# robo-alex/gs-dynamics

Hardware: AMD Instinct MI355X
Metric: fwd+bwd Mpix/s at 100k Gaussians, 4x800^2 views (higher is better)
Workload: dtype f32

## Files before the change

gs-dynamics_amd/csrc/gsr_binning.hip:

```cpp
#include "gsr_common.h"

namespace gsr_binning {

#define SCAN_THREADS 1024
#define SCAN_ITEMS 8
__global__ __launch_bounds__(SCAN_THREADS) void scan_exclusive_kernel(const uint32_t* __restrict__ in,
                                                                      uint32_t* __restrict__ out, uint32_t n,
                                                                      uint32_t* __restrict__ total_out) {
  __shared__ uint32_t wave_tot[SCAN_THREADS / GSR_WAVE];
  __shared__ uint32_t carry_s;
  const int tid = threadIdx.x, lane = tid & 63, wv = tid >> 6;
  if (tid == 0) carry_s = 0;
  __syncthreads();
  const uint32_t per_round = SCAN_THREADS * SCAN_ITEMS;
  for (uint32_t base = 0; base < n; base += per_round) {
    uint32_t v[SCAN_ITEMS];
    uint32_t first = base + (uint32_t)tid * SCAN_ITEMS;
    uint32_t sum = 0;
#pragma unroll
    for (int k = 0; k < SCAN_ITEMS; ++k) {
      uint32_t idx = first + k;
      v[k] = idx < n ? in[idx] : 0u;
      sum += v[k];
    }
// ... 660 lines not shown
  __syncthreads();
  uint32_t before = 0, total = 0;
#pragma unroll
  for (int w = 0; w < GSR_BLOCK / 64; ++w) { if (w < wv) before += s_w[w]; total += s_w[w]; }
  uint32_t* __restrict__ words = vw.block_hist;
  if (tid == 0) __hip_atomic_store(&words[blockIdx.x], 0x80000000u | total, __ATOMIC_RELAXED, __HIP_MEMORY_SCOPE_AGENT);
  if (wv == 0) {
    uint32_t mine = 0;
    if (lane < (int)blockIdx.x) {
      uint32_t w;
      do { w = __hip_atomic_load(&words[lane], __ATOMIC_RELAXED, __HIP_MEMORY_SCOPE_AGENT); } while (!(w & 0x80000000u));
      mine = w & 0x7fffffffu;
    }
#pragma unroll
    for (int k = 32; k >= 1; k >>= 1) mine += __shfl_xor(mine, k, 64);
    if (lane == 0) s_base = mine;
  }
  __syncthreads();
  const uint32_t start = s_base + before + inc - run, cap = vw.D;
  if (t < T) vw.ranges[t] = make_uint2(min(start, cap), min(start + run, cap));
}

__device__ __forceinline__ void bin_scan_view(const GsrBinViews& tab, const GsrBinView& vw, int prefixed, uint32_t* s_wave, uint32_t* s_carry) {
  const int T = tab.T, Ts = gsr_bin_stride(T), rows = tab.rows, tid = threadIdx.x, lane = tid & 63, wv = tid >> 6;
  uint32_t* __restrict__ m = vw.tile_rows;
  const uint32_t cap = vw.D;
  if (tid == 0) *s_carry = 0;
  __syncthreads();
  for (int q0 = 0; q0 < Ts / 4; q0 += BIN_THREADS) {
    const int q = q0 + tid;
    const bool live = q < Ts / 4;
    uint4 tot = make_uint4(0u, 0u, 0u, 0u);
    if (live) {
      if (prefixed) tot = *reinterpret_cast<const uint4*>(m + (size_t)rows * Ts + 4 * q);
      else {
        for (int r0 = 0; r0 < rows; r0 += BIN_ROW_CHUNK) {
          uint4 v[BIN_ROW_CHUNK];
#pragma unroll
          for (int r = 0; r < BIN_ROW_CHUNK; ++r)
            v[r] = r0 + r < rows ? *reinterpret_cast<const uint4*>(m + (size_t)(r0 + r) * Ts + 4 * q) : make_uint4(0u, 0u, 0u, 0u);
#pragma unroll
          for (int r = 0; r < BIN_ROW_CHUNK; ++r)
            if (r0 + r < rows) {
              *reinterpret_cast<uint4*>(m + (size_t)(r0 + r) * Ts + 4 * q) = tot;
              tot.x += v[r].x; tot.y += v[r].y; tot.z += v[r].z; tot.w += v[r].w;
            }
        }
      }
    }
    const uint32_t mine = tot.x + tot.y + tot.z + tot.w;
    uint32_t inc = mine;
#pragma unroll
    for (int d = 1; d < 64; d <<= 1) {
      const uint32_t o = __shfl_up(inc, d, 64);
      if (lane >= d) inc += o;
    }
    if (lane == 63) s_wave[wv] = inc;
    __syncthreads();
    uint32_t start = *s_carry + inc - mine;
    for (int w = 0; w < wv; ++w) start += s_wave[w];
    if (live) {
      const uint32_t c[4] = {tot.x, tot.y, tot.z, tot.w};
      uint32_t st_ = start;
#pragma unroll
      for (int k = 0; k < 4; ++k) {
        if (4 * q + k < T) vw.ranges[4 * q + k] = make_uint2(min(st_, cap), min(st_ + c[k], cap));
        st_ += c[k];
      }
    }
    __syncthreads();
    if (tid == BIN_THREADS - 1) *s_carry = start + mine;
    __syncthreads();
  }
}

__global__ __launch_bounds__(BIN_THREADS) void bin_scan_kernel(GsrBinViews tab, int prefixed) {
  __shared__ uint32_t s_wave[BIN_THREADS / 64];
  __shared__ uint32_t s_carry;
  const GsrBinView& vw = tab.v[blockIdx.x];
  if (vw.shares_lists) return;
  bin_scan_view(tab, vw, prefixed, s_wave, &s_carry);
}

__global__ __launch_bounds__(BIN_THREADS) void bin_emit_kernel(int P, GsrBinViews tab, int order_wgs, int items_per_wg) {
  extern __shared__ uint32_t s_cur[];
  if ((int)blockIdx.x >= tab.rows) {
    __shared__ TileOrderLds L;
    if (blockIdx.y == 0) tile_order_body(tab, items_per_wg, (int)blockIdx.x - tab.rows, L);
    return;
  }
  (void)order_wgs;
  __shared__ uint2 s_big[BIN_BIG_MAX];
  __shared__ uint64_t s_bigkey[BIN_BIG_MAX];
  __shared__ uint32_t s_nbig;
  const GsrBinView& vw = tab.v[blockIdx.y];
  const int T = tab.T, Ts = gsr_bin_stride(T), gx = tab.gx, tid = threadIdx.x, lane = tid & 63, wv = tid >> 6;
  const int g0 = (int)blockIdx.x * GSR_BIN_G;
  if (vw.shares_lists) return;
  const uint32_t cap = vw.D;
  const uint32_t* __restrict__ row = vw.tile_rows + (size_t)blockIdx.x * Ts;
  const uint32_t* __restrict__ cut = vw.depth_cut;
  const bool cut_l = cut && tab.cut_lds;
  const uint32_t* s_cut = s_cur + T;
  const uint32_t* s_cc = s_cur + 2 * T;
  const int gxc = (gx + 3) >> 2;
  if (cut_l)
    for (int t = tid; t < T; t += BIN_THREADS) s_cur[T + t] = cut[t];
  auto cut_at = [&](uint32_t t) { return cut_l ? s_cut[t] : cut[t]; };
  auto behind_all = [&](uint2 r, uint32_t dbits) {
    const uint32_t x0 = (r.x & 0xffffu) >> 2, y0 = (r.x >> 16) >> 2, x1 = ((r.y & 0xffffu) - 1u) >> 2, y1 = ((r.y >> 16) - 1u) >> 2;
    uint32_t m = 0u;
    for (uint32_t y = y0; y <= y1; ++y)
      for (uint32_t x = x0; x <= x1; ++x) m = max(m, s_cc[y * gxc + x]);
    return dbits > m;
  };
  uint64_t* __restrict__ dg = vw.dg[0];
  uint2 rc[BIN_PER_THREAD], ek[BIN_PER_THREAD];
#pragma unroll
  for (int q = 0; q < BIN_PER_THREAD; ++q) {
    const int g = g0 + tid * BIN_PER_THREAD + q;
    rc[q] = make_uint2(0u, 0u); ek[q] = rc[q];
    if (g < P) { rc[q] = vw.rect[g]; ek[q] = vw.ekey[g]; }
  }
  if (tid == 0) s_nbig = 0;
  for (int t = tid; t < T; t += BIN_THREADS) s_cur[t] = vw.ranges[t].x + row[t];
  __syncthreads();
  if (cut_l) {
    const int gyc = (T / gx + 3) >> 2;
    for (int c = tid; c < gxc * gyc; c += BIN_THREADS) {
      const int cx = c % gxc, cy = c / gxc;
      uint32_t m = 0u;
      for (int y = 4 * cy; y < min(4 * cy + 4, T / gx); ++y)
        for (int x = 4 * cx; x < min(4 * cx + 4, gx); ++x) m = max(m, s_cut[y * gx + x]);
      s_cur[2 * T + c] = m;
    }
    __syncthreads();
  }
#pragma unroll
  for (int q = 0; q < BIN_PER_THREAD; ++q) {
    const BinGauss b = bin_gauss(rc[q], ek[q].y);
    if (b.area == 0u) continue;
    if (cut_l && behind_all(rc[q], ek[q].x)) continue;
    const uint64_t key = ((uint64_t)ek[q].x << 32) | (uint32_t)(g0 + tid * BIN_PER_THREAD + q);
    if (b.area > BIN_BIG_AREA) {
      const uint32_t slot = atomicAdd(&s_nbig, 1u);
      if (slot < BIN_BIG_MAX) { s_big[slot] = rc[q]; s_bigkey[slot] = key; continue; }
    }
    const uint32_t dbits = ek[q].x;
    bin_for_tiles(b, gx, [&](uint32_t t) {
      if (cut && dbits > cut_at(t)) return;
      const uint32_t slot = atomicAdd(&s_cur[t], 1u);
      if (slot < cap) dg[slot] = key;
    });
  }
  __syncthreads();
  const uint32_t nbig = min(s_nbig, (uint32_t)BIN_BIG_MAX);
  for (uint32_t i = wv; i < nbig; i += BIN_THREADS / 64) {
    const BinGauss b = bin_gauss(s_big[i], 0u);
    const uint64_t key = s_bigkey[i];
    for (uint32_t k = lane; k < b.area; k += 64) {
      const uint32_t t = bin_tile_of(b, k, gx);
      if (cut && (uint32_t)(key >> 32) > cut_at(t)) continue;
      const uint32_t slot = atomicAdd(&s_cur[t], 1u);
      if (slot < cap) dg[slot] = key;
    }
  }
}

__global__ __launch_bounds__(GSR_BLOCK) void tile_ranges_kernel(GsrBinViews tab, int cur) {
  const GsrBinView& vw = tab.v[blockIdx.y];
  const uint32_t* __restrict__ tkey = vw.tkey[cur];
  uint2* __restrict__ ranges = vw.ranges;
  const uint32_t D = bin_entries(vw);
  uint32_t i = blockIdx.x * GSR_BLOCK + threadIdx.x;
  if (i >= D) return;
  uint32_t t = tkey[i];
  if (i == 0) ranges[t].x = 0;
  else {
    uint32_t pt = tkey[i - 1];
    if (pt != t) { ranges[pt].y = i; ranges[t].x = i; }
  }
  if (i == D - 1) ranges[t].y = D;
}


template <typename PTR>
__device__ __forceinline__ void tile_sort_network(PTR a, uint32_t n, int tid, const uint32_t NT = GSR_BLOCK) {
  uint32_t lg = 1;
  while ((1u << lg) < n) ++lg;
  const uint32_t npairs = (1u << lg) >> 1;
  for (uint32_t lk = 1; lk <= lg; ++lk) {
    const uint32_t k = 1u << lk, hk = k >> 1;
    for (uint32_t p = tid; p < npairs; p += NT) {
      const uint32_t base = (p >> (lk - 1)) << lk, off = p & (hk - 1);
      const uint32_t l = base + off, r = base + (k - 1 - off);
      if (r < n) {
        uint64_t x = a[l], y = a[r];
        if (y < x) { a[l] = y; a[r] = x; }
      }
    }
    __syncthreads();
    for (int lj = (int)lk - 2; lj >= 0; --lj) {
      const uint32_t j = 1u << lj;
      for (uint32_t p = tid; p < npairs; p += NT) {
        const uint32_t l = ((p >> lj) << (lj + 1)) + (p & (j - 1)), r = l + j;
        if (r < n) {
          uint64_t x = a[l], y = a[r];
          if (y < x) { a[l] = y; a[r] = x; }
        }
      }
      __syncthreads();
    }
  }
}

template <int M>
__device__ __forceinline__ uint32_t gsr_lane_xor(uint32_t v) {
  if constexpr (M == 1) return (uint32_t)__builtin_amdgcn_update_dpp(0, (int)v, 0xB1, 0xf, 0xf, true);
  else if constexpr (M == 2) return (uint32_t)__builtin_amdgcn_update_dpp(0, (int)v, 0x4E, 0xf, 0xf, true);
  else if constexpr (M == 3) return (uint32_t)__builtin_amdgcn_update_dpp(0, (int)v, 0x1B, 0xf, 0xf, true);
  else if constexpr (M == 7) return (uint32_t)__builtin_amdgcn_update_dpp(0, (int)v, 0x141, 0xf, 0xf, true);
  else if constexpr (M == 15) return (uint32_t)__builtin_amdgcn_update_dpp(0, (int)v, 0x140, 0xf, 0xf, true);
  else if constexpr (M == 8) return (uint32_t)__builtin_amdgcn_update_dpp(0, (int)v, 0x128, 0xf, 0xf, true);
  else if constexpr (M < 32) return (uint32_t)__builtin_amdgcn_ds_swizzle((int)v, (M << 10) | 0x1F);
  else return (uint32_t)__shfl_xor((int)v, M, 64);
}
template <int V> struct gsr_log2 { static constexpr int value = 1 + gsr_log2<(V >> 1)>::value; };
template <> struct gsr_log2<1> { static constexpr int value = 0; };
template <int MASK, int NR>
__device__ __forceinline__ void wave_sort_step(uint64_t (&x)[NR], int lane) {
  constexpr int LR = gsr_log2<NR>::value;
  constexpr int R = MASK & (NR - 1), L = MASK >> LR;
  constexpr int HB = MASK >= 1024 ? 1024 : MASK >= 512 ? 512 : MASK >= 256 ? 256 : MASK >= 128 ? 128 : MASK >= 64 ? 64 : MASK >= 32 ? 32 : MASK >= 16 ? 16 : MASK >= 8 ? 8 : MASK >= 4 ? 4 : MASK >= 2 ? 2 : 1;
  if constexpr (L == 0) {
#pragma unroll
    for (int r = 0; r < NR; ++r) {
      if ((r & HB) == 0) {
        const uint64_t a = x[r], b = x[r ^ R];
        const bool sw = b < a;
        x[r] = sw ? b : a;
        x[r ^ R] = sw ? a : b;
      }
    }
  } else {
    uint64_t y[NR];
#pragma unroll
    for (int r = 0; r < NR; ++r) {
      const uint64_t src = x[r ^ R];
      y[r] = ((uint64_t)gsr_lane_xor<L>((uint32_t)(src >> 32)) << 32) | gsr_lane_xor<L>((uint32_t)src);
    }
    const bool upper = (lane & (HB >> LR)) != 0;
#pragma unroll
    for (int r = 0; r < NR; ++r) {
      const bool take = (y[r] < x[r]) != upper;
      x[r] = take ? y[r] : x[r];
    }
  }
}
template <int LK, int NR>
__device__ __forceinline__ void wave_sort_stage(uint64_t (&x)[NR], int lane) {
  static_assert(LK <= 11, "the half-cleaner steps below stop at stride 512");
  wave_sort_step<(1 << LK) - 1, NR>(x, lane);
  if constexpr (LK >= 11) wave_sort_step<512, NR>(x, lane);
  if constexpr (LK >= 10) wave_sort_step<256, NR>(x, lane);
  if constexpr (LK >= 9) wave_sort_step<128, NR>(x, lane);
  if constexpr (LK >= 8) wave_sort_step<64, NR>(x, lane);
  if constexpr (LK >= 7) wave_sort_step<32, NR>(x, lane);
  if constexpr (LK >= 6) wave_sort_step<16, NR>(x, lane);
  if constexpr (LK >= 5) wave_sort_step<8, NR>(x, lane);
  if constexpr (LK >= 4) wave_sort_step<4, NR>(x, lane);
  if constexpr (LK >= 3) wave_sort_step<2, NR>(x, lane);
  if constexpr (LK >= 2) wave_sort_step<1, NR>(x, lane);
}
template <int NR>
__device__ __forceinline__ void wave_sort_tile(const uint64_t* __restrict__ seg, uint32_t* __restrict__ out, uint32_t n, int lane) {
  uint64_t x[NR];
#pragma unroll
  for (int r = 0; r < NR; ++r) { const uint32_t e = (uint32_t)(r * 64 + lane); x[r] = e < n ? seg[e] : ~0ull; }
  wave_sort_stage<1, NR>(x, lane); wave_sort_stage<2, NR>(x, lane); wave_sort_stage<3, NR>(x, lane);
  wave_sort_stage<4, NR>(x, lane); wave_sort_stage<5, NR>(x, lane); wave_sort_stage<6, NR>(x, lane);
  if constexpr (NR >= 2) wave_sort_stage<7, NR>(x, lane);
  if constexpr (NR >= 4) wave_sort_stage<8, NR>(x, lane);
  if constexpr (NR >= 8) wave_sort_stage<9, NR>(x, lane);
  if constexpr (NR >= 16) wave_sort_stage<10, NR>(x, lane);
  if constexpr (NR >= 32) wave_sort_stage<11, NR>(x, lane);
  const uint32_t e0 = (uint32_t)lane * NR;
  if constexpr (NR >= 4) {
    if ((((uintptr_t)out) & 15u) == 0 && e0 + NR <= n) {
#pragma unroll
      for (int r = 0; r < NR; r += 4)
        *reinterpret_cast<uint4*>(out + e0 + r) = make_uint4((uint32_t)x[r], (uint32_t)x[r + 1], (uint32_t)x[r + 2], (uint32_t)x[r + 3]);
      return;
    }
  }
#pragma unroll
  for (int r = 0; r < NR; ++r) if (e0 + r < n) out[e0 + r] = (uint32_t)x[r];
}

template <int RCAP, int NW = 4>
struct TileSortLds {
  union {
    struct { uint32_t key[2][RCAP]; uint32_t val[2][RCAP]; } r;
    uint64_t net[2 * RCAP];
  };
  uint32_t whist[NW][256];
  uint32_t wtot[4];
  uint32_t diff;
};

template <int RCAP, int NW>
__device__ __forceinline__ int tile_radix_sort(TileSortLds<RCAP, NW>& L, uint32_t n, int tid) {
  constexpr int NT = 64 * NW;
  const int lane = tid & 63, wv = tid >> 6;
  const uint32_t q = ((n + (uint32_t)NT - 1u) / (uint32_t)NT) << 6;
  const uint32_t wstart = min(n, (uint32_t)wv * q), wstop = min(n, wstart + q);
  const uint32_t diff = L.diff;
  int cur = 0;
  for (int shift = 0; shift < 32; shift += 8) {
    if (((diff >> shift) & 0xffu) == 0u) continue;
    const uint32_t* __restrict__ kin = L.r.key[cur];
    const uint32_t* __restrict__ vin = L.r.val[cur];
    uint32_t* __restrict__ kout = L.r.key[cur ^ 1];
    uint32_t* __restrict__ vout = L.r.val[cur ^ 1];
    for (int i = tid; i < NW * 256; i += NT) (&L.whist[0][0])[i] = 0;
    __syncthreads();
    for (uint32_t i = wstart + lane; i < wstop; i += 64) atomicAdd(&L.whist[wv][(kin[i] >> shift) & 0xffu], 1u);
    __syncthreads();
    {
      uint32_t c[NW], tot = 0;
      if (tid < 256) {
#pragma unroll
        for (int w = 0; w < NW; ++w) { c[w] = L.whist[w][tid]; tot += c[w]; }
      }
      uint32_t inc = tot;
#pragma unroll
      for (int d = 1; d < 64; d <<= 1) {
        const uint32_t o = __shfl_up(inc, d, 64);
        if (lane >= d) inc += o;
      }
      if (tid < 256 && lane == 63) L.wtot[wv] = inc;
      __syncthreads();
      if (tid < 256) {
        uint32_t base = inc - tot;
        for (int w = 0; w < wv; ++w) base += L.wtot[w];
#pragma unroll
        for (int w = 0; w < NW; ++w) { L.whist[w][tid] = base; base += c[w]; }
      }
    }
    __syncthreads();
    volatile uint32_t* wbase = L.whist[wv];
    for (uint32_t i0 = wstart; i0 < wstop; i0 += 64) {
      const uint32_t i = i0 + lane;
      const bool valid = i < wstop;
      uint32_t key = 0, val = 0;
      if (valid) { key = kin[i]; val = vin[i]; }
      const uint32_t digit = (key >> shift) & 0xffu;
      const uint64_t peers = match_peers(digit, valid, 8);
      const uint32_t rank = (uint32_t)__popcll(peers & gsr_lanemask_lt());
      uint32_t pos = 0;
      if (valid) pos = wbase[digit] + rank;
      __builtin_amdgcn_wave_barrier();
      if (valid && rank == 0) wbase[digit] = pos + (uint32_t)__popcll(peers);
      __builtin_amdgcn_wave_barrier();
      if (valid) { kout[pos] = key; vout[pos] = val; }
    }
    __syncthreads();
    cur ^= 1;
  }
  return cur;
}

template <int RCAP, int NW>
__device__ __forceinline__ void tile_sort_long_ticket(const GsrBinViews& tab, int cur, uint32_t ticket);

#ifndef TS_W32_WAVES
#define TS_W32_WAVES 5
#endif
#ifndef TS_MIN_WAVES
#define TS_MIN_WAVES 7
#endif
template <int RCAP, int MODE = 0, int NW = 4>
__global__ __launch_bounds__(64 * NW, (RCAP <= 1024 || MODE == 2) ? TS_MIN_WAVES : (MODE == 3 ? TS_W32_WAVES : 1)) void tile_sort_kernel(GsrBinViews tab, int cur) {
  const int tid = threadIdx.x;
  if constexpr (MODE == 3) {
    const uint32_t n_long3 = tab.queue[6], n_mid = tab.queue[3];
    const uint32_t ticket = n_long3 + blockIdx.x * 4u + (uint32_t)(tid >> 6);
    if (ticket >= n_mid) return;
    const uint4 ord = tab.order[ticket];
    const GsrBinView& vw = tab.v[__builtin_amdgcn_readfirstlane(ord.w)];
    if (vw.shares_lists) return;
    const uint32_t n = __builtin_amdgcn_readfirstlane(ord.z - ord.y);
    wave_sort_tile<32>(vw.dg[cur] + ord.y, vw.point_list + ord.y, n, tid & 63);
    return;
  }
  const uint32_t n_busy = tab.queue[4], n_long = tab.queue[6];
  if (MODE == 2 || (MODE == 0 && blockIdx.x >= n_long)) {
    const uint32_t first = (MODE == 2 && tab.wave_cap == 2048) ? tab.queue[3] : n_long;
    const uint32_t ticket = first + (MODE == 2 ? blockIdx.x : blockIdx.x - n_long) * 4u + (uint32_t)(tid >> 6);
    if (ticket >= n_busy) return;
    const uint4 ord = tab.order[ticket];
    const GsrBinView& vw = tab.v[__builtin_amdgcn_readfirstlane(ord.w)];
    if (vw.shares_lists) return;
    const uint32_t n = __builtin_amdgcn_readfirstlane(ord.z - ord.y);
    const uint64_t* seg = vw.dg[cur] + ord.y;
    uint32_t* out = vw.point_list + ord.y;
    if (n <= 64) wave_sort_tile<1>(seg, out, n, tid & 63);
    else if (n <= 128) wave_sort_tile<2>(seg, out, n, tid & 63);
    else if (n <= 256) wave_sort_tile<4>(seg, out, n, tid & 63);
    else if (n <= 512) wave_sort_tile<8>(seg, out, n, tid & 63);
    else wave_sort_tile<16>(seg, out, n, tid & 63);
    return;
  }
  if constexpr (MODE == 1) {
    const uint32_t n_mine = tab.wave_cap == 512 ? tab.queue[2] : n_long;
    for (uint32_t ticket = blockIdx.x; ticket < n_mine; ticket += gridDim.x) {
      tile_sort_long_ticket<RCAP, NW>(tab, cur, ticket);
      __syncthreads();
    }
  } else if constexpr (MODE != 2) {
    if (blockIdx.x >= n_long) return;
    if (RCAP <= 1024 && tab.vlong_launch && blockIdx.x < tab.queue[2]) return;
    tile_sort_long_ticket<RCAP, NW>(tab, cur, blockIdx.x);
  }
}

template <int RCAP, int NW>
__device__ __forceinline__ void tile_sort_long_ticket(const GsrBinViews& tab, int cur, uint32_t ticket) {
  __shared__ TileSortLds<RCAP, NW> L;
  constexpr uint32_t NT = 64 * NW;
  const int tid = threadIdx.x;
  const uint4 ord = tab.order[ticket];
  const GsrBinView& vw = tab.v[__builtin_amdgcn_readfirstlane(ord.w)];
  if (vw.shares_lists) return;
  uint64_t* __restrict__ dg = vw.dg[cur];
  uint32_t* __restrict__ point_list = vw.point_list;
  const uint2 rg = make_uint2(ord.y, ord.z);
  const uint32_t n = rg.y - rg.x;
  if (n == 0) return;
  uint64_t* seg = dg + rg.x;
  if (n == 1) {
    if (tid == 0) point_list[rg.x] = (uint32_t)seg[0];
  } else if (n <= (uint32_t)RCAP) {
    if (tid == 0) L.diff = 0;
    __syncthreads();
    const uint32_t k0 = (uint32_t)(seg[0] >> 32);
    uint32_t d = 0;
    for (uint32_t i = tid; i < n; i += NT) {
      const uint64_t e = seg[i];
      const uint32_t k = (uint32_t)(e >> 32);
      L.r.key[0][i] = k; L.r.val[0][i] = (uint32_t)e;
      d |= k ^ k0;
    }
    if (d) atomicOr(&L.diff, d);
    __syncthreads();
    const int cur = tile_radix_sort(L, n, tid);
    {
      uint32_t* __restrict__ kk = L.r.key[cur];
      uint32_t* __restrict__ vv = L.r.val[cur];
      bool long_run = false;
      for (uint32_t i = tid; i + 1 < n; i += NT) {
        if (kk[i] == kk[i + 1] && (i == 0 || kk[i - 1] != kk[i])) {
          uint32_t j = i + 1;
          while (j + 1 < n && kk[j + 1] == kk[i] && j - i < 32u) ++j;
          if (j + 1 < n && kk[j + 1] == kk[i]) { long_run = true; continue; }
          for (uint32_t a = i + 1; a <= j; ++a) {
            const uint32_t x = vv[a];
            uint32_t b = a;
            while (b > i && vv[b - 1] > x) { vv[b] = vv[b - 1]; --b; }
            vv[b] = x;
          }
        }
      }
      if (__syncthreads_or(long_run ? 1 : 0)) {
        uint64_t e[(RCAP + NT - 1) / NT];
#pragma unroll
        for (int u = 0; u < (RCAP + NT - 1) / NT; ++u) {
          const uint32_t i = (uint32_t)u * NT + tid;
          e[u] = i < n ? (((uint64_t)kk[i] << 32) | vv[i]) : 0ull;
        }
        __syncthreads();
#pragma unroll
        for (int u = 0; u < (RCAP + NT - 1) / NT; ++u) {
          const uint32_t i = (uint32_t)u * NT + tid;
          if (i < n) L.net[i] = e[u];
        }
        __syncthreads();
        tile_sort_network(L.net, n, tid, NT);
        for (uint32_t i = tid; i < n; i += NT) point_list[rg.x + i] = (uint32_t)L.net[i];
        return;
      }
    }
    for (uint32_t i = tid; i < n; i += NT) point_list[rg.x + i] = L.r.val[cur][i];
  } else if (n <= 2u * (uint32_t)RCAP) {
    for (uint32_t i = tid; i < n; i += NT) L.net[i] = seg[i];
    __syncthreads();
    tile_sort_network(L.net, n, tid, NT);
    for (uint32_t i = tid; i < n; i += NT) point_list[rg.x + i] = (uint32_t)L.net[i];
  } else {
    __syncthreads();
    tile_sort_network((volatile uint64_t*)seg, n, tid, NT);
    for (uint32_t i = tid; i < n; i += NT) point_list[rg.x + i] = (uint32_t)seg[i];
  }
}

__global__ __launch_bounds__(GSR_BLOCK) void copy_tile_state_kernel(int T, int n_order, const uint2* __restrict__ src_ranges,
                                                                    const uint4* __restrict__ src_order, const uint32_t* __restrict__ src_queue,
                                                                    uint2* __restrict__ ranges, uint4* __restrict__ order, uint32_t* __restrict__ queue) {
  const int i = blockIdx.x * GSR_BLOCK + threadIdx.x;
  if (i < T) ranges[i] = src_ranges[i];
  if (i < n_order) order[i] = src_order[i];
  if (i < 9) queue[i] = (i == 4 || i == 6 || i == 7) ? src_queue[i] : 0u;
}

}
using namespace gsr_binning;

int gsr_launch_shared_lists(const GsrBinViews& tab_in, int P, uint32_t D, const uint2* owner_ranges, const uint4* owner_order,
                            const uint32_t* owner_queue, uint2* ranges, uint4* order, uint32_t* queue, hipStream_t st) {
  GsrBinViews tab = tab_in;
  tab.v[0].shares_lists = 1;
  { GSR_PROF("emit_entries", st);
    hipLaunchKernelGGL(emit_entries_kernel, dim3(D / GSR_RADIX_EPB + 1u, 1), dim3(GSR_BLOCK), 0, st, P, tab, 0, 1); }
  GSR_HIP_CHECK(hipGetLastError());
  { GSR_PROF("copy_tile_state", st);
    hipLaunchKernelGGL(copy_tile_state_kernel, dim3((tab.T + GSR_BLOCK - 1) / GSR_BLOCK), dim3(GSR_BLOCK), 0, st, tab.T, tab.T, owner_ranges,
                       owner_order, owner_queue, ranges, order, queue); }
  GSR_HIP_CHECK(hipGetLastError());
  return 0;
}

int gsr_launch_scan_exclusive(const uint32_t* in, uint32_t* out, uint32_t n, uint32_t* total_out, hipStream_t st) {
  { GSR_PROF("scan", st);
  hipLaunchKernelGGL(scan_exclusive_kernel, dim3(1), dim3(SCAN_THREADS), 0, st, in, out, n, total_out); }
  GSR_HIP_CHECK(hipGetLastError());
  return 0;
}

static int ceil_log2_u32(uint32_t n) {
  int b = 0;
  while (((uint64_t)1 << b) < n) ++b;
  return b;
}

static size_t bin_lds_limit() {
  static const size_t v = [] {
    int dev = 0, a = 0;
    if (hipGetDevice(&dev) == hipSuccess && hipDeviceGetAttribute(&a, hipDeviceAttributeMaxSharedMemoryPerBlock, dev) == hipSuccess && a > 0) return (size_t)a;
    return (size_t)(64 << 10);
  }();
  return v;
}
static size_t bin_lds_static() {
  static const size_t v = [] {
    hipFuncAttributes a{}, b{};
    size_t m = 0;
    if (hipFuncGetAttributes(&a, reinterpret_cast<const void*>(bin_emit_kernel)) == hipSuccess) m = a.sharedSizeBytes;
    if (hipFuncGetAttributes(&b, reinterpret_cast<const void*>(bin_count_kernel)) == hipSuccess && b.sharedSizeBytes > m) m = b.sharedSizeBytes;
    return m ? m : (size_t)(52 << 10);
  }();
  return v;
}
bool gsr_rows_path_ok(int T) {
  const char* e = getenv("GSR_RADIX_BINNING");
  const bool radix_only = e && *e && atoi(e) != 0;
  return !radix_only && T > 0 && T <= GSR_BIN_MAX_T && bin_lds_static() + sizeof(uint32_t) * (size_t)T <= bin_lds_limit();
}
int gsr_launch_binning(const GsrBinViews& tab_in, int P, hipStream_t st) {
  if (tab_in.V <= 0 || tab_in.T <= 0) return 0;
  GsrBinViews tab = tab_in;
  uint32_t maxD = 0, maxblk = 0;
  for (int v = 0; v < tab.V; ++v) { maxD = tab.v[v].D > maxD ? tab.v[v].D : maxD; maxblk = tab.v[v].nblocks > maxblk ? tab.v[v].nblocks : maxblk; }
  const char* force = getenv("GSR_TILE_SORT_RCAP");
  const bool big = force ? (force[0] == '4') : (maxD / (uint32_t)tab.T > 600u);
  tab.wave_cap = big ? 2048 : 512;
  {
    static uint32_t* hint = [] { uint32_t* p = nullptr; if (hipHostMalloc((void**)&p, 64, hipHostMallocMapped | hipHostMallocCoherent) != hipSuccess) return (uint32_t*)nullptr; *p = 1u; return p; }();
    tab.vlong_out = hint;
    tab.vlong_launch = (!hint || __atomic_load_n(hint, __ATOMIC_RELAXED) != 0u) ? 1 : 0;
  }
  int cur = 0;
  bool order_done = false;
  bool any_cut = false;
  for (int v = 0; v < tab.V; ++v) any_cut = any_cut || tab.v[v].depth_cut != nullptr;
  const size_t coarse = (size_t)((tab.gx + 3) / 4) * (size_t)((tab.T / tab.gx + 3) / 4);
  tab.cut_lds = (any_cut && bin_lds_static() + sizeof(uint32_t) * (2 * (size_t)tab.T + coarse) <= bin_lds_limit()) ? 1 : 0;
  const size_t lds = sizeof(uint32_t) * (tab.cut_lds ? 2 * (size_t)tab.T + coarse : (size_t)tab.T);
  const bool rows_path = tab.rows > 0 && gsr_rows_path_ok(tab.T) && maxD > 0 && P > 0;
  if (rows_path) {
    { GSR_PROF("bin_count", st);
      hipLaunchKernelGGL(bin_count_kernel, dim3(tab.rows, tab.V), dim3(BIN_THREADS), lds, st, P, tab);
    }
    GSR_HIP_CHECK(hipGetLastError());
    const int prefixed = tab.rows > BIN_DIRECT_ROWS ? 1 : 0;
    const int col_wgs = (gsr_bin_stride(tab.T) + GSR_BLOCK - 1) / GSR_BLOCK;
    const bool chained = prefixed && col_wgs <= 64;
    if (chained) {
      GSR_PROF("bin_colprefix", st);
      hipLaunchKernelGGL(bin_colprefix_scan_kernel, dim3(col_wgs, tab.V), dim3(GSR_BLOCK), 0, st, tab);
    } else if (prefixed) {
      GSR_PROF("bin_colprefix", st);
      hipLaunchKernelGGL(bin_colprefix_kernel, dim3(col_wgs, tab.V), dim3(GSR_BLOCK), 0, st, tab);
    }
    GSR_HIP_CHECK(hipGetLastError());
    const int n_items = tab.V * ((tab.T + 1023) / 1024);
    if (!chained) {
      GSR_PROF("bin_scan", st);
      hipLaunchKernelGGL(bin_scan_kernel, dim3(tab.V), dim3(BIN_THREADS), 0, st, tab, prefixed);
    }
    GSR_HIP_CHECK(hipGetLastError());
    int order_wgs = 0, per_wg = 1;
    {
      order_wgs = n_items < ORD_MAX_WG ? n_items : ORD_MAX_WG;
      if (order_wgs < 1) order_wgs = 1;
      per_wg = (n_items + order_wgs - 1) / order_wgs;
      if (per_wg < 1) per_wg = 1;
      order_wgs = (n_items + per_wg - 1) / per_wg;
      if (order_wgs < 1) order_wgs = 1;
      order_done = true;
    }
    { GSR_PROF("bin_emit", st);
      hipLaunchKernelGGL(bin_emit_kernel, dim3(tab.rows + order_wgs, tab.V), dim3(BIN_THREADS), lds, st, P, tab, order_wgs, per_wg); }
    GSR_HIP_CHECK(hipGetLastError());
  } else if (maxD == 0 || P <= 0) {
    for (int v = 0; v < tab.V; ++v) GSR_HIP_CHECK(hipMemsetAsync(tab.v[v].ranges, 0, sizeof(uint2) * (size_t)tab.T, st));
  } else {
    const int tbits = ceil_log2_u32((uint32_t)tab.T);
    const int npass = (tbits + 7) / 8;
    const int bpp = npass ? (tbits + npass - 1) / npass : 0;
    { GSR_PROF("emit_entries", st);
    const int bits0 = npass ? (tbits < bpp ? tbits : bpp) : 1;
    hipLaunchKernelGGL(emit_entries_kernel, dim3(maxD / GSR_RADIX_EPB + 1u, tab.V), dim3(GSR_BLOCK), 0, st, P, tab, 0, bits0); }
    GSR_HIP_CHECK(hipGetLastError());
    for (int pass = 0; pass < npass; ++pass) {
      const int shift = pass * bpp;
      const int bits = (tbits - shift) < bpp ? (tbits - shift) : bpp;
      if (pass > 0) {
        GSR_PROF("radix_hist", st);
        hipLaunchKernelGGL(radix_hist_kernel, dim3(maxblk, tab.V), dim3(GSR_BLOCK), 0, st, tab, cur, shift, bits);
      }
      GSR_HIP_CHECK(hipGetLastError());
      const int prescanned = maxblk >= GSR_COLSCAN_MIN_BLOCKS ? 1 : 0;
      if (prescanned) {
        GSR_PROF("radix_colscan", st);
        hipLaunchKernelGGL(radix_colscan_kernel, dim3(1u << bits, tab.V), dim3(1024), 0, st, tab, bits);
      }
      GSR_HIP_CHECK(hipGetLastError());
      { GSR_PROF("radix_scatter", st);
      hipLaunchKernelGGL(radix_scatter_kernel, dim3(maxblk, tab.V), dim3(GSR_BLOCK), 0, st, tab, cur, shift, bits, prescanned,
                         pass == npass - 1 ? 1 : 0); }
      GSR_HIP_CHECK(hipGetLastError());
      cur ^= 1;
    }
    if (npass == 0) {
      GSR_PROF("tile_ranges", st);
      hipLaunchKernelGGL(tile_ranges_kernel, dim3((maxD + GSR_BLOCK - 1) / GSR_BLOCK, tab.V), dim3(GSR_BLOCK), 0, st, tab, cur);
    }
    GSR_HIP_CHECK(hipGetLastError());
  }
  if (!order_done)
    if (int rc = gsr_launch_tile_order(tab, st)) return rc;
  if (maxD > 0 && P > 0) {
    { GSR_PROF("tile_sort", st);
    if (big) {
      hipLaunchKernelGGL((tile_sort_kernel<2048, 2>), dim3((tab.V * tab.T + 3) / 4), dim3(GSR_BLOCK), 0, st, tab, cur);
      if (tab.wave_cap == 2048) hipLaunchKernelGGL((tile_sort_kernel<2048, 3>), dim3((tab.V * tab.T + 3) / 4), dim3(GSR_BLOCK), 0, st, tab, cur);
      const int g1 = tab.V * tab.T < 512 ? tab.V * tab.T : 512;
      hipLaunchKernelGGL((tile_sort_kernel<4096, 1, 8>), dim3(g1), dim3(512), 0, st, tab, cur);
    } else
      {
        const bool small_lds = !(force && force[0] == '2');
        if (small_lds) {
          hipLaunchKernelGGL(tile_sort_kernel<1024>, dim3(tab.V * tab.T), dim3(GSR_BLOCK), 0, st, tab, cur);
          if (tab.vlong_launch) hipLaunchKernelGGL((tile_sort_kernel<4096, 1, 16>), dim3(64), dim3(1024), 0, st, tab, cur);
        } else hipLaunchKernelGGL(tile_sort_kernel<2048>, dim3(tab.V * tab.T), dim3(GSR_BLOCK), 0, st, tab, cur);
      } }
    GSR_HIP_CHECK(hipGetLastError());
  }
  return 0;
}

int gsr_launch_tile_order(const GsrBinViews& tab, hipStream_t st) {
  { GSR_PROF("tile_order", st);
    const int n_items = tab.V * ((tab.T + 1023) / 1024);
    int wgs = n_items < ORD_MAX_WG ? n_items : ORD_MAX_WG;
    if (wgs < 1) wgs = 1;
    const int per_wg = (n_items + wgs - 1) / wgs;
    wgs = per_wg > 0 ? (n_items + per_wg - 1) / per_wg : 1;
    hipLaunchKernelGGL(tile_order_kernel, dim3(wgs < 1 ? 1 : wgs), dim3(1024), 0, st, tab, per_wg > 0 ? per_wg : 1); }
  GSR_HIP_CHECK(hipGetLastError());
  return 0;
}
```

Baseline: 5564.

## Sort tiles up to 1024 entries with a four-wave bitonic network

For tiles with at most 1024 entries in the RCAP=1024, four-wave configuration, the radix sort through LDS is replaced by a register bitonic sort. Each wave sorts 256 keys in registers, and three cross-wave merge steps exchange data through a new LDS union member. This avoids the multiple radix passes with histogram and scatter work, at the cost of a full bitonic network even on partly filled tiles. The branch placement with __syncthreads inside the helper is uniform per block, so barrier correctness relies on every thread taking the same path.

```diff
diff --git a/gs-dynamics_amd/csrc/gsr_binning.hip b/gs-dynamics_amd/csrc/gsr_binning.hip
--- a/gs-dynamics_amd/csrc/gsr_binning.hip
+++ b/gs-dynamics_amd/csrc/gsr_binning.hip
@@ -986,6 +986,7 @@
   union {
     struct { uint32_t key[2][RCAP]; uint32_t val[2][RCAP]; } r;
     uint64_t net[2 * RCAP];
+    uint64_t xch[2][4][RCAP / 4];
   };
   uint32_t whist[NW][256];
   uint32_t wtot[4];
@@ -1108,6 +1109,55 @@
   }
 }
 
+template <int MASK>
+__device__ __forceinline__ void wg_sort_cross_step(uint64_t (&x)[4], uint64_t (*buf)[256], uint32_t w, int lane, uint32_t n, bool live) {
+  constexpr uint32_t PW = MASK >> 8;
+  constexpr bool MIRROR = (MASK & 255) != 0;
+  if (live) {
+#pragma unroll
+    for (int r = 0; r < 4; ++r) buf[w][r * 64 + lane] = x[r];
+  }
+  __syncthreads();
+  if (live && (w ^ PW) * 256u < n) {
+    const bool upper = (w & (MASK >= 512 ? 2u : 1u)) != 0;
+#pragma unroll
+    for (int r = 0; r < 4; ++r) {
+      const uint64_t y = buf[w ^ PW][(MIRROR ? (r ^ 3) : r) * 64 + (MIRROR ? (lane ^ 63) : lane)];
+      const bool take = (y < x[r]) != upper;
+      x[r] = take ? y : x[r];
+    }
+  }
+}
+__device__ __forceinline__ void wave_sort_clean128(uint64_t (&x)[4], int lane) {
+  wave_sort_step<128, 4>(x, lane); wave_sort_step<64, 4>(x, lane); wave_sort_step<32, 4>(x, lane); wave_sort_step<16, 4>(x, lane);
+  wave_sort_step<8, 4>(x, lane); wave_sort_step<4, 4>(x, lane); wave_sort_step<2, 4>(x, lane); wave_sort_step<1, 4>(x, lane);
+}
+__device__ __forceinline__ void tile_sort_four_waves(uint64_t (*xch)[4][256], const uint64_t* __restrict__ seg, uint32_t* __restrict__ out, uint32_t n, int tid) {
+  const int lane = tid & 63;
+  const uint32_t w = (uint32_t)__builtin_amdgcn_readfirstlane(tid >> 6), base = w * 256u;
+  const bool live = base < n;
+  uint64_t x[4];
+  if (live) {
+#pragma unroll
+    for (int r = 0; r < 4; ++r) { const uint32_t e = base + (uint32_t)(r * 64 + lane); x[r] = e < n ? seg[e] : ~0ull; }
+    wave_sort_stage<1, 4>(x, lane); wave_sort_stage<2, 4>(x, lane); wave_sort_stage<3, 4>(x, lane); wave_sort_stage<4, 4>(x, lane);
+    wave_sort_stage<5, 4>(x, lane); wave_sort_stage<6, 4>(x, lane); wave_sort_stage<7, 4>(x, lane); wave_sort_stage<8, 4>(x, lane);
+  }
+  wg_sort_cross_step<511>(x, xch[0], w, lane, n, live);
+  if (live) wave_sort_clean128(x, lane);
+  wg_sort_cross_step<1023>(x, xch[1], w, lane, n, live);
+  wg_sort_cross_step<256>(x, xch[0], w, lane, n, live);
+  if (live) {
+    wave_sort_clean128(x, lane);
+    const uint32_t e0 = base + (uint32_t)lane * 4u;
+    if ((((uintptr_t)out) & 15u) == 0 && e0 + 4u <= n) *reinterpret_cast<uint4*>(out + e0) = make_uint4((uint32_t)x[0], (uint32_t)x[1], (uint32_t)x[2], (uint32_t)x[3]);
+    else {
+#pragma unroll
+      for (int r = 0; r < 4; ++r) if (e0 + r < n) out[e0 + r] = (uint32_t)x[r];
+    }
+  }
+}
+
 template <int RCAP, int NW>
 __device__ __forceinline__ void tile_sort_long_ticket(const GsrBinViews& tab, int cur, uint32_t ticket) {
   __shared__ TileSortLds<RCAP, NW> L;
@@ -1124,6 +1174,8 @@
   uint64_t* seg = dg + rg.x;
   if (n == 1) {
     if (tid == 0) point_list[rg.x] = (uint32_t)seg[0];
+  } else if (RCAP == 1024 && NW == 4 && n <= 1024u) {
+    if constexpr (RCAP == 1024 && NW == 4) tile_sort_four_waves(L.xch, seg, point_list + rg.x, n, tid);
   } else if (n <= (uint32_t)RCAP) {
     if (tid == 0) L.diff = 0;
     __syncthreads();
```

Result: no change. 5632 (median of 6 runs) (+1.2%).
